# flanglet/kanzi-cpp

Measured on AMD Instinct MI355X. Metric: encode+decode MB/s on the synthetic stand-in for silesia.tar (bit-exact), higher is better.
Workload: dtype u8

## Files before the change

kanzi-cpp_amd/csrc/bwt_fwd.hip:

```cpp
#include "common.hpp"
#include "stages.hpp"
#include "bwt_common.hpp"

#include <cstdlib>
#include <cstring>
#include <algorithm>
#include <cmath>
#include "prims.hpp"
#include <chrono>
#include <vector>

namespace knz {

constexpr u32 SM_TS = 1792;
constexpr u32 SM_WIN = 2048;
constexpr u32 SM_G = 256;
constexpr u32 MED_CAP = 8192;
constexpr u32 MED_LO_CAP = 2048;
constexpr u32 SUPER_CAP = 8192;
constexpr int GATHER_THREADS = 512;
constexpr u32 GATHER_ROWS = 16;
static_assert(MED_CAP <= GATHER_ROWS * GATHER_THREADS, "k_bwt_f_gather_desc judges a medium group from one batch of loads");
constexpr u32 LARGE_OS_MIN = 1000000;
constexpr u32 NO_BIT = 0x7FFFFFFFu;

struct FwdView {
    const u32* base;
    int nBlocks;
    u32 total;
    u32* SA;
    u32* ISA;
    u64* ISA2;
    u32 round;
    u32* K;
    u32* gbits;
    u32* gnew;
    u32* counters;
    const u32* ovr;
    const u32* rtbits;
    uint2* medStage;
    uint2* verdictNow;
    const uint2* verdictWas;
};

constexpr u32 VERDICT_WHOLE = 1, VERDICT_PLAIN = 2;
__host__ __device__ __forceinline__ u32 verdict_word(u32 round, u32 status, u32 members) { return (round << 24) | (status << 16) | members; }
static_assert(MED_CAP < (1u << 16), "verdict_word keeps a medium group's size in 16 bits");

enum FwdCounter : u32 {
    CNT_SMALL_LEFT = 0,
    CNT_MED = 1,
    CNT_LARGE = 2,
    CNT_LARGE_MEMBERS = 3,
    CNT_RUN = 4,
    CNT_RUN_MEMBERS = 5,
    CNT_RUN_LONGEST = 6,
    CNT_SUPER = 7,
    CNT_RUNS = 8,
    CNT_MED_LO = 9,
    CNT_STAT_SMALL = 10,
    CNT_STAT_SMALL_GROUPS = 11,
    CNT_STAT_MED = 12,
    CNT_TIED = 13,
    CNT_PROBE_CAND = 14,
    CNT_LINKED = 14,
    CNT_LINK_TIED = 15,
    CNT_STAT_MED_GROUPS = 16,
    CNT_STAT_UNSPLIT = 17,
    CNT_STAT_UNSPLIT_MEMBERS = 18,
    CNT_STAT_MAJ = 19,
    CNT_STAT_MAJ_MEMBERS = 20,
    CNT_STAT_ASLEEP = 21,
    CNT_STAT_ASLEEP_MEMBERS = 22,
    CNT_ROUND_SLOTS = 24,
    CNT_PROBE_SLOTS = 2,
    CNT_LONGEST_BLOCK = 32,
    CNT_NSYM = 33,
};

constexpr u32 LAB_BITS = 28;
constexpr u64 LAB_MASK = (1ull << LAB_BITS) - 1ull;

__device__ __forceinline__ u32 lab_old(const FwdView& v, u32 q, u32 bb)
{
    if (v.ISA2 == nullptr) return v.ISA[q];
    const u64 e = v.ISA2[q];
    const u32 rel = ((u32)(e >> 56) == v.round && v.round != 0) ? (u32)((e >> LAB_BITS) & LAB_MASK) : (u32)(e & LAB_MASK);
    return bb + rel;
}
__device__ __forceinline__ u32 lab_cur(const FwdView& v, u32 q, u32 bb)
{
    if (v.ISA2 == nullptr) return v.ISA[q];
    return bb + (u32)(v.ISA2[q] & LAB_MASK);
}
__device__ __forceinline__ void lab_set(const FwdView& v, u32 p, u32 bb, u32 lab, u32 was)
{
    if (v.ISA2 == nullptr) { v.ISA[p] = lab; return; }
#ifdef KNZ_EMU
    if (v.round != 0 && lab_old(v, p, bb) != was) {
        fprintf(stderr, "lab_set: round %u position %u: was %u, label %u\n", v.round, p, was, lab_old(v, p, bb));
        abort();
    }
#endif
    const u64 nw = (u64)(lab - bb), ow = (v.round == 0) ? nw : (u64)(was - bb);
    v.ISA2[p] = nw | (ow << LAB_BITS) | ((u64)v.round << 56);
}

__device__ __forceinline__ u32 gather_key(const FwdView& v, u32 gp, u32 h, u32 blkBase, u32 blkEnd)
{
    const u32 q = gp + h;
    return (q < blkEnd) ? lab_old(v, q, blkBase) - blkBase + 1u : 0u;
}

__device__ __forceinline__ void classify_child(const FwdView& v, uint2* __restrict__ medNext, uint2* __restrict__ largeNext, u32 start, u32 size, u32& surv)
{
    if (size > MED_CAP) {
        const u32 at = atomicAdd(&v.counters[CNT_LARGE], 1u);
        largeNext[at] = make_uint2(start, size);
        atomicAdd(&v.counters[CNT_LARGE_MEMBERS], size);
    } else if (size > SM_G) {
        v.medStage[start >> 8] = make_uint2(start, size);
    } else if (size > 1) {
        surv = 1;
    }
}

// ... 1742 lines not shown
}

__global__ __launch_bounds__(256) void k_bwt_f_run_members(const u32* __restrict__ moff, u32 nRuns, u32 M, const u64* __restrict__ sKey, int kbits, int hbits,
                                                           u32 nsym, u64* __restrict__ mkeys)
{
    __shared__ u32 sOff[2048 + 1];
    __shared__ u32 sFirst;
    const u32 j0 = blockIdx.x * 2048u;
    if (j0 >= M) return;
    if (threadIdx.x == 0) {
        u32 lo = 0, hi = nRuns;
        while (hi - lo > 1) { const u32 mid = (lo + hi) >> 1; if (moff[mid] <= j0) lo = mid; else hi = mid; }
        sFirst = lo;
    }
    __syncthreads();
    const u32 k0 = sFirst;
    for (u32 i = threadIdx.x; i <= 2048u; i += 256) sOff[i] = (k0 + i < nRuns) ? moff[k0 + i] : 0xFFFFFFFFu;
    __syncthreads();
#pragma unroll
    for (int q = 0; q < 8; q++) {
        const u32 j = j0 + (u32)q * 256u + threadIdx.x;
        if (j >= M) continue;
        u32 lo = 0, hi = 2048;
        while (hi - lo > 1) { const u32 mid = (lo + hi) >> 1; if (sOff[mid] <= j) lo = mid; else hi = mid; }
        if (sOff[hi] <= j) lo = hi;
        const u32 k = k0 + lo;
        const u64 key = sKey[k];
        const u64 cls = key >> (kbits + 1);
        const bool above = (key >> kbits) & 1ull;
        const u64 Rr = (u64)nsym + (u64)(j - sOff[lo]);
        const u64 hiK = above ? ((1ull << hbits) - 1ull - Rr) : Rr;
        mkeys[j] = (((cls << hbits) | hiK) << 32) | (u64)k;
    }
}

__global__ __launch_bounds__(256) void k_bwt_f_run_expand(const u64* __restrict__ mkeys, u32 M, const u64* __restrict__ sKey, const u32* __restrict__ sE,
                                                          int kbits, int hbits, u64* __restrict__ keys, u32* __restrict__ vals, u32* __restrict__ Rout)
{
    const u32 j = blockIdx.x * 256 + threadIdx.x;
    if (j >= M) return;
    const u64 mk = mkeys[j];
    const u32 k = (u32)mk;
    const u64 ch = mk >> 32;
    const u64 hiK = ch & ((1ull << hbits) - 1ull);
    const u64 rk = sKey[k];
    const bool above = (rk >> kbits) & 1ull;
    const u64 T = rk & ((1ull << kbits) - 1ull);
    const u32 Rr = (u32)(above ? ((1ull << hbits) - 1ull - hiK) : hiK);
    keys[j] = (ch << kbits) | T;
    vals[j] = sE[k] - Rr;
    Rout[j] = Rr;
}

__global__ __launch_bounds__(256) void k_bwt_f_run_flags(const u64* __restrict__ keys, u32 M, unsigned long long* __restrict__ bits64)
{
    const u32 j = blockIdx.x * 256 + threadIdx.x;
    const u64 k = (j < M) ? keys[j] : 0ull;
    u32 klo = (u32)__shfl_up((int)(u32)k, 1u, 64), khi = (u32)__shfl_up((int)(u32)(k >> 32), 1u, 64);
    u64 kp = ((u64)khi << 32) | klo;
    if ((threadIdx.x & 63) == 0 && j > 0 && j < M) kp = keys[j - 1];
    const bool f = (j >= M) || (j == 0) || (k != kp);
    const unsigned long long m = __ballot(f);
    if ((threadIdx.x & 63) == 0) bits64[j >> 6] = m;
}

__global__ __launch_bounds__(256) void k_bwt_f_run_place(FwdView v, const uint2* __restrict__ desc, const u32* __restrict__ loff, u32 M, int kbits, const u64* __restrict__ keys,
                                                         const u32* __restrict__ vals, const u32* __restrict__ bits, const u32* __restrict__ winLastIncl,
                                                         const u32* __restrict__ winFirstInclRev, u32 nWin, uint2* __restrict__ largeNext, const u32* __restrict__ memberR,
                                                         u32* __restrict__ ovr, u32* __restrict__ rtbits, const u32* __restrict__ lbase)
{
    __shared__ SmWindow W;
    __shared__ ClassAgg A;
    const int tid = (int)threadIdx.x;
    const u32 jb = blockIdx.x * 256u;
    const u32 win = jb / SM_WIN, j0 = win * SM_WIN;
    agg_init(A);
    if (tid < 64) {
        const u32 w = bits[(j0 >> 5) + (u32)tid];
        W.bw[tid] = w;
        int pm = w ? (tid * 32 + 31 - __clz((int)w)) : -1;
        u32 sm = w ? (u32)(tid * 32 + __ffs((int)w) - 1) : NO_BIT;
        for (int o = 1; o < 64; o <<= 1) {
            const int t = __shfl_up(pm, (unsigned)o, 64);
            if (tid >= o) pm = t > pm ? t : pm;
            const u32 u = (u32)__shfl_down((int)sm, (unsigned)o, 64);
            if (tid + o < 64) sm = u < sm ? u : sm;
        }
        int pex = __shfl_up(pm, 1u, 64);
        if (tid == 0) pex = -1;
        u32 sex = (u32)__shfl_down((int)sm, 1u, 64);
        if (tid == 63) sex = NO_BIT;
        W.prevSet[tid] = pex;
        W.nextSet[tid] = sex;
    }
    __syncthreads();
    const u32 j = jb + (u32)tid;
    u32 surv = 0, mySlot = 0, hLocal = 0, hSize = 0;
    int hKind = -1;
    bool setBit = false;
    if (j < M) {
        const u32 i = j - j0;
        const u32 w = i >> 5, bit = i & 31;
        const u32 lowmask = (bit == 31) ? 0xFFFFFFFFu : ((2u << bit) - 1u);
        const u32 word = W.bw[w];
        const u32 m = word & lowmask;
        const int si = m ? (int)(w * 32 + 31 - (u32)__clz((int)m)) : W.prevSet[w];
// ... 73 lines not shown
        u32 word = 0, have = 0;
#pragma unroll
        for (u32 k = 0; k < 4; k++) {
            const u32 q = 4 * w + k;
            if (q >= qLo && q < qHi) {
                const u32 rr = q - qLo;
                const u32 r = rr + (rr >= r0 ? 1u : 0u);
                const u32 p = SA[bb + r] - bb;
                word |= (u32)s[p - 1] << (8 * k);
                have |= 1u << k;
            }
        }
        if (have == 0xF && al) reinterpret_cast<u32*>(d)[w] = word;
        else for (u32 k = 0; k < 4; k++) if ((have >> k) & 1) d[4 * w + k] = (u8)(word >> (8 * k));
    }
    if (blockIdx.x == 0 && threadIdx.x == 0) {
        d[hdr] = s[n - 1];
        const u32 st = n / (u32)chunks;
        const u32 step = ((u32)chunks * st == n) ? st : st + 1;
        const u32 logNbChunks = (u32)ilog2_u32((u32)chunks);
        d[0] = (u8)((logNbChunks << 2) | (pIndexSize - 1));
        u32 idx = 1;
        for (int k = 0; k < chunks; k++) {
            const u32 prim = lab_cur(fv, bb + (u32)k * step, bb) - bb;
            for (int sh = (int)(pIndexSize - 1) * 8; sh >= 0; sh -= 8) d[idx++] = (u8)(prim >> sh);
        }
        newLen[b] = hdr + n;
    }
}

__global__ __launch_bounds__(256) void k_bwt_f_med_flags(const uint2* __restrict__ stage, u32 nSlots, u32* __restrict__ flags)
{
    const u32 i = blockIdx.x * 256 + threadIdx.x;
    if (i >= nSlots) return;
    const u32 n = stage[i].y;
    flags[i] = (n != 0 && n <= MED_LO_CAP) ? 1u : 0u;
    flags[nSlots + i] = (n > MED_LO_CAP) ? 1u : 0u;
}

__global__ __launch_bounds__(256) void k_bwt_f_med_compact(uint2* __restrict__ stage, u32 nSlots, const u32* __restrict__ prefix, uint2* __restrict__ medNext,
                                                           u32 at, u32* __restrict__ idxLo, u32 atLo, u32* __restrict__ idxHi, u32 atHi, u32* __restrict__ nLoOut)
{
    const u32 i = blockIdx.x * 256 + threadIdx.x;
    if (i >= nSlots) return;
    const u32 nLo = prefix[nSlots];
    if (i == 0) *nLoOut = nLo;
    const uint2 d = stage[i];
    if (d.y == 0) return;
    const u32 pLo = prefix[i], pHi = prefix[nSlots + i] - nLo, g = at + pLo + pHi;
    medNext[g] = d; stage[i] = make_uint2(0u, 0u);
    if (d.y <= MED_LO_CAP) idxLo[atLo + pLo] = g; else idxHi[atHi + pHi] = g;
}

struct FwdTuning { int nsym; int noRunRound; int runFallback; int stats; int link; int plainLabels; int noPack; int noUnsplitSkip; int noGroupSleep; int noMediumFuse; };
static FwdTuning& fwd_tuning()
{
    static FwdTuning t = [] {
        FwdTuning x; x.nsym = 0; x.noRunRound = 0; x.runFallback = 0; x.stats = 0; x.link = 1; x.plainLabels = 0; x.noPack = 0; x.noUnsplitSkip = 0; x.noGroupSleep = 0; x.noMediumFuse = 0;
        if (getenv("KNZ_BWT_PLAIN_LABELS")) x.plainLabels = 1;
        if (getenv("KNZ_BWT_NO_PACK")) x.noPack = 1;
        if (getenv("KNZ_BWT_NO_UNSPLIT_SKIP")) x.noUnsplitSkip = 1;
        if (getenv("KNZ_BWT_NO_GROUP_SLEEP")) x.noGroupSleep = 1;
        if (getenv("KNZ_BWT_NO_MEDIUM_FUSE")) x.noMediumFuse = 1;
        if (const char* e = getenv("KNZ_BWT_LINK")) x.link = atoi(e);
        if (getenv("KNZ_BWT_STATS")) x.stats = 1;
        if (const char* e = getenv("KNZ_BWT_NSYM")) x.nsym = atoi(e);
        if (getenv("KNZ_BWT_NO_RUN_ROUND")) x.noRunRound = 1;
        if (getenv("KNZ_BWT_RUN_FALLBACK")) x.runFallback = 1;
        return x;
    }();
    return t;
}
int bwt_forward_tune(const char* key, int value)
{
    FwdTuning& t = fwd_tuning();
    if (!strcmp(key, "rs_onesweep")) { prims::rs_onesweep_knob().store(value); return 0; }
    if (!strcmp(key, "bwt_nsym")) t.nsym = value;
    else if (!strcmp(key, "bwt_no_run_round")) t.noRunRound = value;
    else if (!strcmp(key, "bwt_run_fallback")) t.runFallback = value;
    else if (!strcmp(key, "bwt_stats")) t.stats = value;
    else if (!strcmp(key, "bwt_link")) t.link = value;
    else if (!strcmp(key, "bwt_plain_labels")) t.plainLabels = value;
    else if (!strcmp(key, "bwt_no_pack")) t.noPack = value;
    else if (!strcmp(key, "bwt_no_unsplit_skip")) t.noUnsplitSkip = value;
    else if (!strcmp(key, "bwt_no_group_sleep")) t.noGroupSleep = value;
    else if (!strcmp(key, "bwt_no_medium_fuse")) t.noMediumFuse = value;
    else return -1;
    return 0;
}

struct FwdScratch {
    u64* keysA; u64* keysB;
    u32* valsA; u32* valsB;
    u32* SA; u32* ISA; u32* K; u64* ISA2;
    u32* t0; u32* t1; u32* t2; u32* t3;
    u32* gbits; u32* gnew; u32* rtbits; u32* ovr; size_t gbitsWords;
    uint2* med[2]; uint2* medStage; uint2* medVerdict[2]; u32* medFlags; u32* medPrefix; u32* medIdxLo; u32* medIdxHi; size_t medSlots; uint2* descInfo; uint2* large[2]; uint2* runList; uint4* superList; u32* ebits;
    u32* loff; u32* lbase;
    u32* survTile;
    u32* linkedTile;
    u32* base;
    u32* counters;
    u32* seg2;
    void* scanTmp;
    void* rsMem;
    u32* byteHist;
    u32* classTab; u32* rbits; u32* rcount; u32* rprefix;
    u32* runPos; u32* runE; u32* runL; u32* sE; u32* rcnt; u32* moff;
    u64* runKeysA; u64* runKeysB; u64* sKey;
    size_t maxRuns;
};

static size_t fwd_align(size_t x) { return (x + 255) & ~(size_t)255; }

static size_t fwd_carve(u8* p, int nBlocks, size_t total, FwdScratch* w, u32 VS)
{
    u8* q = p;
    auto take = [&](size_t sz) { u8* r = q; q += fwd_align(sz); return r; };
    const size_t maxMed = 2 * (total / (SM_G + 1) + 2), maxLarge = total / (MED_CAP + 1) + 2;
    w->gbitsWords = ((total + 64) / 64 + SM_WIN / 64 + 4) * 2 + 128;
    w->keysA = (u64*)take(8 * total); w->keysB = (u64*)take(8 * total);
    w->valsA = (u32*)take(4 * total); w->valsB = (u32*)take(4 * total);
    w->SA = (u32*)take(4 * total); w->ISA = (u32*)take(4 * total); w->K = (u32*)take(4 * total);
    w->ISA2 = (VS <= (1u << LAB_BITS)) ? (u64*)take(8 * total) : (u64*)nullptr;
    w->t0 = (u32*)take(4 * total); w->t1 = (u32*)take(4 * total); w->t2 = (u32*)take(4 * total); w->t3 = (u32*)take(4 * total);
    w->gbits = (u32*)take(4 * w->gbitsWords);
    w->gnew = (u32*)take(4 * w->gbitsWords);
    w->rtbits = (u32*)take(4 * w->gbitsWords);
    w->ovr = (u32*)take(4 * total);
    w->med[0] = (uint2*)take(8 * maxMed); w->med[1] = (uint2*)take(8 * maxMed);
    w->medSlots = total / 256 + 2;
    w->medStage = (uint2*)take(8 * w->medSlots); w->medFlags = (u32*)take(8 * w->medSlots + 64); w->medPrefix = (u32*)take(8 * w->medSlots + 64);
    w->medIdxLo = (u32*)take(4 * maxMed); w->medIdxHi = (u32*)take(4 * maxMed);
    w->medVerdict[0] = (uint2*)take(16 * w->medSlots); w->medVerdict[1] = w->medVerdict[0] + w->medSlots;
    w->large[0] = (uint2*)take(8 * maxLarge); w->large[1] = (uint2*)take(8 * maxLarge);
    w->runList = (uint2*)take(8 * maxMed);
    w->superList = (uint4*)take(16 * maxMed);
    w->descInfo = (uint2*)take(8 * maxMed);
    w->ebits = (u32*)take(4 * w->gbitsWords);
    w->loff = (u32*)take(4 * (maxMed + 1));
    w->lbase = (u32*)take(4 * (maxMed + 1));
    w->survTile = (u32*)take(4 * (total / SM_TS + 64));
    w->linkedTile = (u32*)take(4 * (total / SM_TS + 64));
    w->base = (u32*)take(4ull * (nBlocks + 2));
    w->counters = (u32*)take(256);
    w->byteHist = (u32*)take(1024ull * (nBlocks + 1));
    w->seg2 = (u32*)take(64);
    w->scanTmp = take(prims::scan_tmp_bytes(total + 16));
    w->rsMem = take(prims::rs_ws_bytes(total, nBlocks + 1));
    w->maxRuns = total / 4 + 64;
    w->classTab = (u32*)take(1024ull * (size_t)nBlocks);
    const size_t rw = total / 32 + SM_WIN / 32 + 136;
    w->rbits = (u32*)take(4 * rw); w->rcount = (u32*)take(4 * rw); w->rprefix = (u32*)take(4 * rw);
    w->runPos = (u32*)take(4 * w->maxRuns); w->runE = (u32*)take(4 * w->maxRuns); w->runL = (u32*)take(4 * w->maxRuns);
    w->sE = (u32*)take(4 * w->maxRuns); w->rcnt = (u32*)take(4 * w->maxRuns); w->moff = (u32*)take(4 * w->maxRuns + 64);
    w->runKeysA = (u64*)take(8 * w->maxRuns); w->runKeysB = (u64*)take(8 * w->maxRuns); w->sKey = (u64*)take(8 * w->maxRuns);
    return (size_t)(q - p);
}

size_t bwt_forward_scratch_bytes(int nBlocks, u32 VS, size_t total)
{
    FwdScratch w;
    return fwd_carve(nullptr, nBlocks, total, &w, VS) + 4096;
}

#define GRID1(n) dim3((unsigned)(((n) + 255) / 256)), dim3(256), 0, s

static int bits_for(u64 n, int lo) { while ((1ull << lo) < n) lo++; return lo; }

struct LinkPlan {
    enum Mode { UNTRIED, TRIAL, ON, APPLIED, OFF } mode = UNTRIED;
    int trials = 0; u32 retryH = 0xFFFFFFFFu;
    bool next(u32 h, u32 survMembers, u32 total, u32 linked, u32 tied, bool stats)
    {
        if (mode == TRIAL || mode == APPLIED) {
            const bool paid = linked >= 4096 && tied < linked / 2;
            mode = paid ? ON : OFF;
            if (!paid) retryH = (trials < 2) ? h * 8 : 0xFFFFFFFFu;
            if (stats) fprintf(stderr, "link step: %u members linked, %u of the windows' members still tied after the round -> %s\n", linked, tied, paid ? "on" : "off");
        }
        if (mode == OFF && h >= retryH) mode = UNTRIED;
        if (mode == UNTRIED && survMembers >= total / 8) { mode = TRIAL; trials++; return true; }
        if (mode == ON && survMembers >= total / 64) { mode = APPLIED; return true; }
        return false;
    }
};

struct FwdSort {
    hipStream_t s; const XfStage& st; u32* hp;
    const FwdTuning tune = fwd_tuning();
    BwtView bv; FwdView v; FwdScratch w; size_t maxTotal;
    prims::RsWs rs1;
    u32 total, medSlots, nTiles; int nsym, pbits, kbits;
    bool groupSleep = false;
    u32 h = 1; int cur = 0;
    u64 *keysFree, *keysFree2;
    bool medFuse = false;
    u32 nMedLo = 0;
    u32 nRun, runElems, surv, nMed, nLarge, largeElems, survMembers;
    LinkPlan link; LinkTrial linkTr; std::chrono::steady_clock::time_point statT;
    int fetch(u32 first, u32 n) { return hipMemcpyAsync(hp + first, w.counters + first, 4 * (size_t)n, hipMemcpyDeviceToHost, s) == hipSuccess && hipStreamSynchronize(s) == hipSuccess ? 0 : -1; }
    void merge_bits() { hipLaunchKernelGGL(k_bwt_f_merge_bits, GRID1(total / 32 + 2), w.gbits, w.gnew, total / 32 + 2); }
    void enable_run_tiebits() { if (!v.rtbits) { hipMemsetAsync(w.rtbits, 0, 4 * w.gbitsWords, s); v.ovr = w.ovr; v.rtbits = w.rtbits; } }
    void compact_medium(uint2* dst, u32 at = 0, u32 atLo = 0)
    {
        KScope ks_("k_bwt_f_med_compact");
        hipLaunchKernelGGL(k_bwt_f_med_flags, GRID1(medSlots), w.medStage, medSlots, w.medFlags);
        prims::launch_scan<prims::SCAN_SUM_EXCL>(s, w.medFlags, w.medPrefix, 2 * (size_t)medSlots, nullptr, w.scanTmp, w.counters + CNT_MED);
        hipLaunchKernelGGL(k_bwt_f_med_compact, GRID1(medSlots), w.medStage, medSlots, w.medPrefix, dst, at, w.medIdxLo, atLo, w.medIdxHi, at - atLo, w.counters + CNT_MED_LO);
    }
    void bounds(u32 n, bool last, const u32* bits = nullptr, u32 len = 0, u32 wordsPerWin = 0)
    {
        if (bits) { KScope ks_("k_bwt_f_r0_winsum"); hipLaunchKernelGGL(k_bwt_f_r0_winsum, GRID1(n), bits, len, n, w.t0, w.t2, wordsPerWin); }
        if (last) { KScope ks_("k_bwt_f_scan_max"); prims::launch_scan<prims::SCAN_MAX_INCL>(s, w.t0, w.t1, n, nullptr, w.scanTmp); }
        KScope ks_("k_bwt_f_scan_min"); prims::launch_scan<prims::SCAN_MIN_INCL>(s, w.t2, w.t3, n, nullptr, w.scanTmp);
    }
    template <class KEY, bool HAS_VAL> int sort_one_segment(u32 n, KEY* ka, KEY* kb, u32* va, u32* vb, int loBit, int hiBit, bool oneRead = true)
    {
        hipLaunchKernelGGL(prims::k_rs_one_segment, dim3(1), dim3(64), 0, s, w.seg2, n);
        prims::rs_launch_layout(s, rs1);
        return prims::rs_sort<KEY, HAS_VAL>(s, rs1, ka, kb, va, vb, (size_t)n, loBit, hiBit, oneRead);
    }
    int setup(void* scratch, size_t scratchBytes, BwtSuffixArrays* sa)
    {
        bv.src = st.src; bv.dst = st.dst; bv.len = st.len; bv.cap = st.cap; bv.VS = st.maxLen; bv.nBlocks = st.nBlocks;
        maxTotal = (size_t)st.nBlocks * bv.VS;
        if (fwd_carve(reinterpret_cast<u8*>(scratch), st.nBlocks, maxTotal, &w, bv.VS) > scratchBytes) return -2;
        { KScope ks_("k_bwt_f_bases"); hipLaunchKernelGGL(k_bwt_bases, dim3(1), dim3(64), 0, s, bv, w.base, st.ok, w.counters + CNT_LONGEST_BLOCK, sa ? 1 : 0); }
        hipMemsetAsync(st.newLen, 0, sizeof(u32) * st.nBlocks, s);
        { KScope ks_("k_bwt_f_r0_hist");
          hipMemsetAsync(w.byteHist, 0, 1024ull * st.nBlocks, s);
          hipLaunchKernelGGL(k_bwt_f_bytehist, dim3(64, (unsigned)st.nBlocks), dim3(256), 0, s, bv, w.base, w.byteHist);
          hipLaunchKernelGGL(k_bwt_f_choose_nsym, dim3(1), dim3(256), 0, s, w.byteHist, st.nBlocks, w.counters + CNT_LONGEST_BLOCK, w.counters + CNT_NSYM); }
        if (hipMemcpyAsync(hp, w.base + st.nBlocks, 4, hipMemcpyDeviceToHost, s) != hipSuccess || fetch(CNT_LONGEST_BLOCK, 2)) return -1;
        total = hp[0];
        if (sa) { sa->SA = w.SA; sa->base = w.base; sa->total = total; }
        if (total == 0) return 0;
        v.base = w.base; v.nBlocks = st.nBlocks; v.total = total; v.SA = w.SA; v.ISA = w.ISA; v.K = w.K; v.ISA2 = (w.ISA2 != nullptr && !tune.plainLabels) ? w.ISA2 : (u64*)nullptr;
        v.round = 0; v.gbits = w.gbits; v.gnew = w.gnew; v.counters = w.counters; v.medStage = w.medStage; v.ovr = nullptr; v.rtbits = nullptr;
        v.verdictNow = nullptr; v.verdictWas = nullptr;
        medSlots = (u32)((size_t)total / 256 + 1); nTiles = (total + SM_TS - 1) / SM_TS;
        survMembers = total;
        hipMemsetAsync(w.medStage, 0, 8ull * w.medSlots, s);
        medFuse = v.ISA2 != nullptr && !tune.noMediumFuse;
        groupSleep = !tune.noUnsplitSkip && !tune.noGroupSleep;
        if (groupSleep) hipMemsetAsync(w.medVerdict[0], 0, 16ull * w.medSlots, s);
        pbits = bits_for(hp[CNT_LONGEST_BLOCK], 1);
        const int fit = (64 - pbits) / 8, want = (hp[CNT_NSYM] == 5u) ? 5 : 4;
        nsym = fit < want ? fit : want;
        if (tune.nsym >= 1) nsym = tune.nsym < fit ? tune.nsym : fit;
// ... 23 lines not shown
            if (pass == 0) { TextSrc src; src.src = bv.src; src.P = nsym; src.pbits = pbits; src.shift = pbits; sortPass(src, pass); }
            else { prims::DigitOfKey<u64> src; src.keys = kin; src.shift = pbits + 8 * pass; src.mask = 255u; sortPass(src, pass); }
            std::swap(kin, kout);
        }
        keysFree = kout; keysFree2 = kin;
    }
    int round0_place()
    {
        hipMemsetAsync(w.gbits, 0xFF, 4 * w.gbitsWords, s); hipMemsetAsync(w.gnew, 0, 4 * w.gbitsWords, s);
        hipMemsetAsync(w.counters, 0, 4 * CNT_ROUND_SLOTS, s);
        { KScope ks_("k_bwt_f_r0_flags"); hipLaunchKernelGGL(k_bwt_f_r0_flags, dim3((total + 256 * R0F_ROWS - 1) / (256 * R0F_ROWS)), dim3(256), 0, s, keysFree2, w.base, st.nBlocks, total, nsym, pbits,
                                                             reinterpret_cast<unsigned long long*>(w.gbits)); }
        bounds(nTiles, true, w.gbits, total, SM_TS / 32);
        kbits = bits_for((u64)bv.VS + 2, 1);
        const bool runRound = (2 * kbits + 1) < 64 && !tune.noRunRound;
        { KScope ks_("k_bwt_f_r0_place");
          hipLaunchKernelGGL(k_bwt_f_r0_place_text, dim3(nTiles), dim3(256), 0, s, bv, v, w.t1, w.t3, nTiles, w.large[cur], keysFree2, nsym, pbits, runRound ? w.runList : (uint2*)nullptr);
          merge_bits(); }
        if (fetch(0, CNT_ROUND_SLOTS)) return -1;
        nRun = hp[CNT_RUN]; runElems = hp[CNT_RUN_MEMBERS];
        return 0;
    }
    int run_fallback()
    {
        { KScope ks_("k_bwt_f_run_fallback"); hipLaunchKernelGGL(k_bwt_f_run_fallback, GRID1(nRun), v, w.runList, nRun, w.med[cur], w.large[cur]); }
        nRun = 0; return fetch(0, CNT_ROUND_SLOTS);
    }
    int run_round()
    {
        if (nRun && ((u64)nRun > (1ull << (64 - (2 * kbits + 1))) || tune.runFallback) && run_fallback()) return -1;
        if (!nRun) return 0;
        const u32 nWin = (total + SM_WIN - 1) / SM_WIN;
        { KScope ks_("k_bwt_f_run_ends"); hipLaunchKernelGGL(k_bwt_f_run_ends, dim3(nWin), dim3(256), 0, s, bv, v, reinterpret_cast<u8*>(w.ebits)); }
        bounds(nWin, false, w.ebits, total, SM_WIN / 32);
        hipMemsetAsync(w.classTab, 0xFF, 1024ull * (size_t)st.nBlocks, s);
        { KScope ks_("k_bwt_f_run_classes"); hipLaunchKernelGGL(k_bwt_f_run_classes, GRID1(nRun), bv, v, w.runList, nRun, w.classTab); }
        { KScope ks_("k_bwt_f_run_len"); hipLaunchKernelGGL(k_bwt_f_run_len, dim3(nWin), dim3(256), 0, s, bv, v, w.ebits, w.t3, nWin, w.K, w.classTab, (u32)nsym,
                                                            reinterpret_cast<unsigned long long*>(w.rbits), w.rcount); }
        const u32 nRW = nWin * (SM_WIN / 32);
        { KScope ks_("k_bwt_f_scan_sum"); prims::launch_scan<prims::SCAN_SUM_EXCL>(s, w.rcount, w.rprefix, nRW, nullptr, w.scanTmp, w.counters + CNT_RUNS); }
        { KScope ks_("k_bwt_f_run_compact"); hipLaunchKernelGGL(k_bwt_f_run_compact, GRID1(nRW), w.rbits, w.rprefix, nRW, w.runPos); }
        if (fetch(CNT_RUN_LONGEST, 3)) return -1;
        const u32 nRuns = hp[CNT_RUNS];
        const int hbits = bits_for((u64)hp[CNT_RUN_LONGEST] + 1, 1) + 1;
        const int rbits = bits_for(nRun, 0), idxBits = bits_for(nRuns, 1);
        if (nRuns == 0 || nRuns > w.maxRuns || rbits + hbits > 32 || idxBits + kbits + 1 + rbits > 64) return run_fallback();
        { KScope ks_("k_bwt_f_large_prefix"); hipLaunchKernelGGL(k_bwt_f_large_prefix, dim3(1), dim3(1024), 0, s, w.runList, nRun, w.loff, w.base, st.nBlocks, w.lbase); }
        { KScope ks_("k_bwt_f_run_table"); hipLaunchKernelGGL(k_bwt_f_run_table, GRID1(nRuns), bv, v, w.runPos, nRuns, w.K, w.classTab, kbits, idxBits, w.runKeysA, w.runE, w.runL); }
        const u64* rkSorted;
        { KScope ks_("k_bwt_f_sort_runs");
          rkSorted = sort_one_segment<u64, false>(nRuns, w.runKeysA, w.runKeysB, nullptr, nullptr, idxBits, idxBits + kbits + 1 + rbits) ? w.runKeysB : w.runKeysA; }
        { KScope ks_("k_bwt_f_run_sorted"); hipLaunchKernelGGL(k_bwt_f_run_sorted, GRID1(nRuns), rkSorted, nRuns, idxBits, w.runE, w.runL, (u32)nsym, w.sE, w.sKey, w.rcnt); }
        { KScope ks_("k_bwt_f_scan_sum"); prims::launch_scan<prims::SCAN_SUM_EXCL>(s, w.rcnt, w.moff, nRuns, nullptr, w.scanTmp); }
        { KScope ks_("k_bwt_f_run_members"); hipLaunchKernelGGL(k_bwt_f_run_members, dim3((runElems + 2047) / 2048), dim3(256), 0, s, w.moff, nRuns, runElems, w.sKey, kbits, hbits,
                                                                (u32)nsym, keysFree); }
        u64* rk; u32* rv = w.valsA;
        { KScope ks_("k_bwt_f_sort_members");
          const int r = sort_one_segment<u64, false>(runElems, keysFree, keysFree2, nullptr, nullptr, 32, 32 + hbits + rbits);
          rk = r ? keysFree : keysFree2;
          hipLaunchKernelGGL(k_bwt_f_run_expand, GRID1(runElems), r ? keysFree2 : keysFree, runElems, w.sKey, w.sE, kbits, hbits, rk, rv, w.valsB); }
        u32* mbits = w.ebits; const u32 nWinM = (runElems + SM_WIN - 1) / SM_WIN;
        { KScope ks_("k_bwt_f_large_flags"); hipLaunchKernelGGL(k_bwt_f_run_flags, dim3(nWinM * (SM_WIN / 256)), dim3(256), 0, s, rk, runElems, reinterpret_cast<unsigned long long*>(mbits)); }
        bounds(nWinM, true, mbits, runElems, SM_WIN / 32);
        { KScope ks_("k_bwt_f_large_place");
          hipMemsetAsync(w.rtbits, 0, 4 * w.gbitsWords, s);
          hipLaunchKernelGGL(k_bwt_f_run_place, dim3((runElems + 255) / 256), dim3(256), 0, s, v, w.runList, w.loff, runElems, hbits + kbits, rk, rv, mbits, w.t1, w.t3, nWinM, w.large[cur],
                             w.valsB, w.ovr, w.rtbits, w.lbase);
          v.ovr = w.ovr; v.rtbits = w.rtbits; }
        { KScope ks_("k_bwt_f_merge_bits"); merge_bits(); }
        return 0;
    }
    int probe()
    {
        u32* probeCand = w.medFlags;
        compact_medium(w.med[cur]);
        { KScope ks_("k_bwt_f_probe"); hipLaunchKernelGGL(k_bwt_f_probe_scan, dim3(256), dim3(256), 0, s, v, w.med[cur], (u32)nsym, v.rtbits, probeCand); }
        if (fetch(0, CNT_ROUND_SLOTS)) return -1;
        surv = hp[CNT_SMALL_LEFT]; nMed = hp[CNT_MED]; nMedLo = hp[CNT_MED_LO]; nLarge = hp[CNT_LARGE]; largeElems = hp[CNT_LARGE_MEMBERS];
        if (const u32 nCand = hp[CNT_PROBE_CAND]) {
            enable_run_tiebits();
            hipMemsetAsync(w.counters, 0, 4 * CNT_PROBE_SLOTS, s);
            { KScope ks_("k_bwt_f_probe");
              hipLaunchKernelGGL(k_bwt_f_probe, dim3(std::min<u32>(nCand, 4096)), dim3(512), 0, s, bv, v, w.med[cur], probeCand, nCand, (u32)nsym, w.med[cur ^ 1], w.large[cur], w.ovr, w.rtbits);
              merge_bits(); }
            compact_medium(w.med[cur], nMed, nMedLo);
            if (fetch(0, CNT_MED_LO + 1)) return -1;
            surv |= hp[CNT_SMALL_LEFT]; nMed += hp[CNT_MED]; nMedLo += hp[CNT_MED_LO];
        }
        if (tune.stats) fprintf(stderr, "after round 0 (nsym %d, total %u): run groups %u (%u members); small left %u, medium %u, large %u (%u members)\n",
                                nsym, total, nRun, runElems, surv, nMed, nLarge, largeElems);
        statT = std::chrono::steady_clock::now();
        return 0;
    }
    void link_step()
    {
        KScope ks_("k_bwt_f_link");
        u32* posflag = w.ebits; u32* linked = w.rbits; u32* rev = w.rcount; u32* sufRev = w.rprefix;
        const bool trial = link.mode == LinkPlan::TRIAL; linkTr.n = 0;
        if (trial) { linkTr.blk[linkTr.n++] = 0; if (st.nBlocks >= 5) linkTr.blk[linkTr.n++] = st.nBlocks / 2; if (st.nBlocks >= 3) linkTr.blk[linkTr.n++] = st.nBlocks - 1; }
        const u32 nW = total / 32 + 1;
        hipMemsetAsync(posflag, 0, 4 * (size_t)nW, s);
        hipMemsetAsync(linked, 0, 4 * ((size_t)nTiles * (SM_TS / 32) + 64), s);
        enable_run_tiebits();
        const u32 nTrial = (u32)std::min<u64>((u64)nTiles, ((u64)bv.VS + SM_TS - 1) / SM_TS + 2);
        const dim3 gridL(trial ? nTrial : nTiles, (unsigned)(linkTr.n ? linkTr.n : 1));
        hipLaunchKernelGGL(k_bwt_f_link_small, gridL, dim3(256), 0, s, v, posflag, linked, tune.stats, 1u, w.linkedTile, linkTr);
        hipLaunchKernelGGL(k_bwt_f_link_zeros, GRID1(nW), posflag, nW, rev);
        prims::launch_scan<prims::SCAN_MIN_INCL>(s, rev, sufRev, nW, nullptr, w.scanTmp);
        hipLaunchKernelGGL(k_bwt_f_link_apply, gridL, dim3(256), 0, s, v, posflag, sufRev, nW, linked, h, w.ovr, w.rtbits, 1u, linkTr);
    }
    void sort_small(bool linked)
    {
        KScope ks_("k_bwt_f_sort_small");
        u32* survTile = tune.link ? w.survTile : nullptr;
        if (v.ISA2 && pbits <= 23 && !tune.noPack) hipLaunchKernelGGL(k_bwt_f_small_fused<true>, dim3(nTiles), dim3(256), 0, s, v, h, survTile, tune.stats);
        else if (v.ISA2) hipLaunchKernelGGL(k_bwt_f_small_fused<false>, dim3(nTiles), dim3(256), 0, s, v, h, survTile, tune.stats);
        else hipLaunchKernelGGL(k_bwt_f_sort_small, dim3(nTiles), dim3(256), 0, s, v, survTile);
        if (linked) hipLaunchKernelGGL(k_bwt_f_link_payoff, dim3(1), dim3(256), 0, s, v, w.linkedTile, w.survTile, nTiles, 1u, w.counters + CNT_LINKED, linkTr);
        if (tune.link) prims::launch_scan<prims::SCAN_SUM_EXCL>(s, w.survTile, w.survTile, nTiles, nullptr, w.scanTmp, w.counters + CNT_TIED);
    }
    void sort_medium()
    {
        const int npass = (kbits + 7) / 8, nxt = cur ^ 1;
        if (medFuse) {
            KScope ks_("k_bwt_f_medium_fused"); const int skip = tune.noUnsplitSkip ? 0 : 1; const u32 nMedHi = nMed - nMedLo;
            const auto fuse256 = tune.stats ? k_bwt_f_medium_fused<256, 8, true> : k_bwt_f_medium_fused<256, 8, false>;
            const auto fuse512 = tune.stats ? k_bwt_f_medium_fused<512, 16, true> : k_bwt_f_medium_fused<512, 16, false>;
            if (nMedLo) hipLaunchKernelGGL(fuse256, dim3(std::min<u32>((nMedLo + 7) / 8 * 8, 2048)), dim3(256), 0, s, v, w.med[cur], w.medIdxLo, nMedLo, h, npass, skip, w.med[nxt], w.large[nxt], w.superList);
            if (nMedHi) hipLaunchKernelGGL(fuse512, dim3(std::min<u32>((nMedHi + 7) / 8 * 8, 1024)), dim3(512), 0, s, v, w.med[cur], w.medIdxHi, nMedHi, h, npass, skip, w.med[nxt], w.large[nxt], w.superList);
        } else { KScope ks_("k_bwt_f_sort_medium"); const dim3 gridM(std::min<u32>(nMed, 8192));
          const auto sort256 = tune.stats ? k_bwt_f_sort_medium<256, 8, true> : k_bwt_f_sort_medium<256, 8, false>;
          const auto sort512 = tune.stats ? k_bwt_f_sort_medium<512, 16, true> : k_bwt_f_sort_medium<512, 16, false>;
          hipLaunchKernelGGL(sort256, gridM, dim3(256), 0, s, v, w.med[cur], nMed, npass, SM_G, w.med[nxt], w.large[nxt], w.descInfo, w.superList);
          hipLaunchKernelGGL(sort512, gridM, dim3(512), 0, s, v, w.med[cur], nMed, npass, MED_LO_CAP, w.med[nxt], w.large[nxt], w.descInfo, w.superList); }
        { KScope ks_("k_bwt_f_super"); hipLaunchKernelGGL(k_bwt_f_super, dim3(std::min<u32>(nMed, 512)), dim3(1024), 0, s, v, w.superList, h, npass, w.med[nxt], w.large[nxt]); }
    }
    template <class KEY> void large_keys()
    {
        { KScope ks_("k_bwt_f_large_prefix"); hipLaunchKernelGGL(k_bwt_f_large_prefix, dim3(1), dim3(1024), 0, s, w.large[cur], nLarge, w.loff, w.base, st.nBlocks, w.lbase); }
        KScope ks_("k_bwt_f_large_keys");
        hipLaunchKernelGGL(k_bwt_f_large_keys<KEY>, GRID1(largeElems), v, w.large[cur], nLarge, w.loff, largeElems, h, kbits, reinterpret_cast<KEY*>(keysFree), w.valsA);
    }
    template <class KEY> void sort_large(int lbits)
// ... 78 lines not shown
```

Baseline: 6659.

## Place BWT run members directly by counting instead of radix sorting them

When the longest run is at most 1023, the expansion of run members no longer generates keys and radix-sorts them. It splits the run list into tiles, histograms run lengths per tile, and scans per-segment column offsets across tiles. Each member's output position is then computed directly and written in sorted order. This removes a full 64-bit segmented sort over all run members, at the cost of several small kernels and scans plus extra scratch for tile column tables. The original sort path is kept as a fallback behind a tuning flag and for longer runs.

```diff
diff --git a/kanzi-cpp_amd/csrc/bwt_fwd.hip b/kanzi-cpp_amd/csrc/bwt_fwd.hip
--- a/kanzi-cpp_amd/csrc/bwt_fwd.hip
+++ b/kanzi-cpp_amd/csrc/bwt_fwd.hip
@@ -72,6 +72,7 @@
     CNT_STAT_MAJ_MEMBERS = 20,
     CNT_STAT_ASLEEP = 21,
     CNT_STAT_ASLEEP_MEMBERS = 22,
+    CNT_RUN_TILES = 23,
     CNT_ROUND_SLOTS = 24,
     CNT_PROBE_SLOTS = 2,
     CNT_LONGEST_BLOCK = 32,
@@ -1920,6 +1921,205 @@
     Rout[j] = Rr;
 }
 
+constexpr u32 RUN_TILE = 1024;
+constexpr u32 RUN_ROWS = RUN_TILE / 64;
+constexpr u32 RUN_DIRECT_LMAX = 1023;
+constexpr u32 RUN_COLS = RUN_DIRECT_LMAX + 1;
+constexpr u32 RUN_CH = 256;
+static_assert(RUN_COLS == 4 * 256 && RUN_CH == 256 && RUN_ROWS % 4 == 0, "the kernels below map columns and rows to 256 threads");
+static inline size_t run_tile_slots(size_t maxRuns) { return 2 * (maxRuns / RUN_TILE + 2); }
+
+struct RunTile { u32 k0, k1, a, slot; bool first, last, multi; };
+__device__ __forceinline__ RunTile run_tile(const u32* __restrict__ tileStart, const u32* __restrict__ segStart, u32 nRuns, u32 t)
+{
+    RunTile r;
+    r.k0 = tileStart[t]; r.k1 = tileStart[t + 1]; r.a = segStart[r.k0];
+    r.first = r.k0 == r.a;
+    r.last = r.k1 >= nRuns || segStart[r.k1] == r.k1;
+    r.multi = !(r.first && r.last);
+    r.slot = (r.k1 - r.k0 == RUN_TILE) ? 2u * ((r.k0 + RUN_TILE - 1) / RUN_TILE) : (r.k0 >= RUN_TILE ? 2u * ((r.k0 - 1) / RUN_TILE) + 1u : 1u);
+    return r;
+}
+
+__global__ __launch_bounds__(256) void k_bwt_f_run_seg_marks(const u64* __restrict__ sKey, u32 nRuns, int kbits, u32* __restrict__ segMark)
+{
+    const u32 k = blockIdx.x * 256 + threadIdx.x;
+    if (k >= nRuns) return;
+    segMark[k] = (k > 0 && (sKey[k] >> kbits) == (sKey[k - 1] >> kbits)) ? 0u : k;
+}
+
+__global__ __launch_bounds__(256) void k_bwt_f_run_tile_marks(const u32* __restrict__ segStart, u32 nRuns, u32* __restrict__ tileMark)
+{
+    const u32 k = blockIdx.x * 256 + threadIdx.x;
+    if (k >= nRuns) return;
+    tileMark[k] = ((k - segStart[k]) % RUN_TILE == 0) ? 1u : 0u;
+}
+
+__global__ __launch_bounds__(256) void k_bwt_f_run_tile_starts(const u32* __restrict__ segStart, const u32* __restrict__ tileIdx, u32 nRuns, u32* __restrict__ tileStart)
+{
+    const u32 k = blockIdx.x * 256 + threadIdx.x;
+    if (k >= nRuns) return;
+    const bool mark = (k - segStart[k]) % RUN_TILE == 0;
+    const u32 t = tileIdx[k];
+    if (mark) tileStart[t] = k;
+    if (k + 1 == nRuns) tileStart[t + (mark ? 1u : 0u)] = nRuns;
+}
+
+__global__ __launch_bounds__(256) void k_bwt_f_run_tile_counts(const u32* __restrict__ tileStart, const u32* __restrict__ segStart, const u32* __restrict__ rcnt, u32 nRuns,
+                                                               const u32* __restrict__ nTilesDev, u32 nsym, u32* __restrict__ colTab)
+{
+    __shared__ u32 hist[RUN_COLS];
+    __shared__ u32 wsum[4];
+    const u32 t = blockIdx.x, tid = threadIdx.x;
+    if (t >= *nTilesDev) return;
+    const RunTile T = run_tile(tileStart, segStart, nRuns, t);
+    if (!T.multi) return;
+    for (u32 i = tid; i < RUN_COLS; i += 256) hist[i] = 0;
+    __syncthreads();
+    for (u32 k = T.k0 + tid; k < T.k1; k += 256) { const u32 L = rcnt[k] + nsym - 1u; atomicAdd(&hist[L < RUN_DIRECT_LMAX ? L : RUN_DIRECT_LMAX], 1u); }
+    __syncthreads();
+    u32 x[4], acc = 0;
+#pragma unroll
+    for (u32 i = 0; i < 4; i++) { x[i] = hist[4 * tid + i]; acc += x[i]; }
+    u32 tot;
+    const u32 incl = prims::sc_block_incl<prims::SCAN_SUM_EXCL>(acc, wsum, &tot);
+    u32 ge = tot - (incl - acc);
+    u32* row = colTab + (size_t)T.slot * RUN_COLS;
+#pragma unroll
+    for (u32 i = 0; i < 4; i++) { row[4 * tid + i] = ge; ge -= x[i]; }
+}
+
+__global__ __launch_bounds__(256) void k_bwt_f_run_tile_scan(const u32* __restrict__ tileStart, const u32* __restrict__ segStart, const u64* __restrict__ sKey, u32 nRuns,
+                                                             const u32* __restrict__ nTilesDev, u32 nsym, int kbits, u32* __restrict__ colTab)
+{
+    __shared__ u32 wsum[4];
+    const u32 t0 = blockIdx.x, tid = threadIdx.x, nT = *nTilesDev;
+    if (t0 >= nT) return;
+    const RunTile T0 = run_tile(tileStart, segStart, nRuns, t0);
+    if (!T0.multi || !T0.first) return;
+    const bool above = ((sKey[T0.a] >> kbits) & 1ull) != 0;
+    u32 A[4] = { 0, 0, 0, 0 };
+    for (u32 t = t0; t < nT; t++) {
+        const RunTile T = run_tile(tileStart, segStart, nRuns, t);
+        const u32* row = colTab + (size_t)T.slot * RUN_COLS;
+#pragma unroll
+        for (u32 c = 0; c < 4; c++) A[c] += row[tid + 256 * c];
+        if (T.last) break;
+    }
+    u32 P[4], carry = 0;
+#pragma unroll
+    for (u32 c = 0; c < 4; c++) {
+        if (tid + 256 * c < nsym) A[c] = 0;
+        u32 tot;
+        P[c] = carry + prims::sc_block_incl<prims::SCAN_SUM_EXCL>(A[c], wsum, &tot);
+        carry += tot;
+    }
+    u32 run[4];
+#pragma unroll
+    for (u32 c = 0; c < 4; c++) run[c] = above ? carry - P[c] : P[c] - A[c];
+    for (u32 t = t0; t < nT; t++) {
+        const RunTile T = run_tile(tileStart, segStart, nRuns, t);
+        u32* row = colTab + (size_t)T.slot * RUN_COLS;
+#pragma unroll
+        for (u32 c = 0; c < 4; c++) { const u32 x = row[tid + 256 * c]; row[tid + 256 * c] = run[c]; run[c] += x; }
+        if (T.last) break;
+    }
+}
+
+__global__ __launch_bounds__(256) void k_bwt_f_run_emit(const u32* __restrict__ tileStart, const u32* __restrict__ segStart, const u32* __restrict__ rcnt,
+                                                        const u32* __restrict__ moff, const u64* __restrict__ sKey, const u32* __restrict__ sE, u32 nRuns, u32 M,
+                                                        const u32* __restrict__ nTilesDev, const u32* __restrict__ colTab, u32 nsym, int kbits, int hbits,
+                                                        u64* __restrict__ keys, u32* __restrict__ vals, u32* __restrict__ Rout)
+{
+    __shared__ u32 cnt[RUN_ROWS][RUN_CH];
+    __shared__ u32 colBase[RUN_CH];
+    __shared__ u32 wsum[4];
+    __shared__ u32 sLmax;
+    const u32 t = blockIdx.x, tid = threadIdx.x;
+    if (t >= *nTilesDev) return;
+    const int lane = lane_id();
+    const u32 wave = tid >> 6;
+    const RunTile T = run_tile(tileStart, segStart, nRuns, t);
+    const u32 nRows = (T.k1 - T.k0 + 63) / 64;
+    const u32 segBase = moff[T.a];
+    const u32 tileMembers = (T.k1 < nRuns ? moff[T.k1] : M) - moff[T.k0];
+    const bool above = ((sKey[T.k0] >> kbits) & 1ull) != 0;
+    const u64 hiAll = (1ull << hbits) - 1ull;
+    u32 Lr[RUN_ROWS / 4], rowMax[RUN_ROWS / 4], e[RUN_ROWS / 4];
+    u64 kb[RUN_ROWS / 4];
+    u32 lmax = 0;
+    if (tid == 0) sLmax = 0;
+#pragma unroll
+    for (u32 q = 0; q < RUN_ROWS / 4; q++) {
+        const u32 k = T.k0 + (wave + 4 * q) * 64 + (u32)lane;
+        Lr[q] = 0; e[q] = 0; kb[q] = 0;
+        if (k < T.k1) {
+            const u64 key = sKey[k];
+            Lr[q] = rcnt[k] + nsym - 1u;
+            if (Lr[q] > RUN_DIRECT_LMAX) Lr[q] = RUN_DIRECT_LMAX;
+            e[q] = sE[k];
+            kb[q] = ((key >> (kbits + 1)) << (hbits + kbits)) | (key & ((1ull << kbits) - 1ull));
+        }
+        rowMax[q] = wave_max(Lr[q]);
+        lmax = rowMax[q] > lmax ? rowMax[q] : lmax;
+    }
+    __syncthreads();
+    if (lane == 0) atomicMax(&sLmax, lmax);
+    __syncthreads();
+    const u32 Lmax = sLmax;
+    u32 carry = 0;
+    for (u32 c0 = nsym; c0 <= Lmax; c0 += RUN_CH) {
+        for (u32 i = tid; i < nRows * RUN_CH; i += 256) (&cnt[0][0])[i] = 0;
+        __syncthreads();
+#pragma unroll
+        for (u32 q = 0; q < RUN_ROWS / 4; q++)
+            if (Lr[q] >= c0) atomicAdd(&cnt[wave + 4 * q][Lr[q] - c0 < RUN_CH ? Lr[q] - c0 : RUN_CH - 1], 1u);
+        __syncthreads();
+#pragma unroll
+        for (u32 q = 0; q < RUN_ROWS / 4; q++) {
+            const u32 row = wave + 4 * q;
+            if (row >= nRows) break;
+            u32 x[4], acc = 0;
+#pragma unroll
+            for (u32 i = 0; i < 4; i++) { x[i] = cnt[row][4 * lane + i]; acc += x[i]; }
+            const u32 incl = wave_incl_scan(acc);
+            const u32 tot = (u32)__shfl((int)incl, 63, 64);
+            u32 ge = tot - (incl - acc);
+#pragma unroll
+            for (u32 i = 0; i < 4; i++) { cnt[row][4 * lane + i] = ge; ge -= x[i]; }
+        }
+        __syncthreads();
+        u32 colRuns = 0;
+        for (u32 row = 0; row < nRows; row++) { const u32 x = cnt[row][tid]; cnt[row][tid] = colRuns; colRuns += x; }
+        if (T.multi) {
+            colBase[tid] = (c0 + tid < RUN_COLS) ? colTab[(size_t)T.slot * RUN_COLS + c0 + tid] : 0u;
+        } else {
+            u32 tot;
+            const u32 P = carry + prims::sc_block_incl<prims::SCAN_SUM_EXCL>(colRuns, wsum, &tot);
+            colBase[tid] = above ? tileMembers - P : P - colRuns;
+            carry += tot;
+        }
+        __syncthreads();
+#pragma unroll
+        for (u32 q = 0; q < RUN_ROWS / 4; q++) {
+            const u32 row = wave + 4 * q;
+            if (row >= nRows) break;
+            const u32 Rend = rowMax[q] < c0 + RUN_CH - 1 ? rowMax[q] : c0 + RUN_CH - 1;
+            for (u32 R = c0; R <= Rend; R++) {
+                const bool alive = Lr[q] >= R;
+                const unsigned long long m = __ballot(alive);
+                const u32 j = segBase + colBase[R - c0] + cnt[row][R - c0] + (u32)__popcll(m & __lanemask_lt());
+                if (alive && j < M) {
+                    keys[j] = kb[q] | ((above ? hiAll - (u64)R : (u64)R) << kbits);
+                    vals[j] = e[q] - R;
+                    Rout[j] = R;
+                }
+            }
+        }
+        __syncthreads();
+    }
+}
+
 __global__ __launch_bounds__(256) void k_bwt_f_run_flags(const u64* __restrict__ keys, u32 M, unsigned long long* __restrict__ bits64)
 {
     const u32 j = blockIdx.x * 256 + threadIdx.x;
@@ -2099,16 +2299,17 @@
     if (d.y <= MED_LO_CAP) idxLo[atLo + pLo] = g; else idxHi[atHi + pHi] = g;
 }
 
-struct FwdTuning { int nsym; int noRunRound; int runFallback; int stats; int link; int plainLabels; int noPack; int noUnsplitSkip; int noGroupSleep; int noMediumFuse; };
+struct FwdTuning { int nsym; int noRunRound; int runFallback; int stats; int link; int plainLabels; int noPack; int noUnsplitSkip; int noGroupSleep; int noMediumFuse; int runSort; };
 static FwdTuning& fwd_tuning()
 {
     static FwdTuning t = [] {
-        FwdTuning x; x.nsym = 0; x.noRunRound = 0; x.runFallback = 0; x.stats = 0; x.link = 1; x.plainLabels = 0; x.noPack = 0; x.noUnsplitSkip = 0; x.noGroupSleep = 0; x.noMediumFuse = 0;
+        FwdTuning x; x.nsym = 0; x.noRunRound = 0; x.runFallback = 0; x.stats = 0; x.link = 1; x.plainLabels = 0; x.noPack = 0; x.noUnsplitSkip = 0; x.noGroupSleep = 0; x.noMediumFuse = 0; x.runSort = 0;
         if (getenv("KNZ_BWT_PLAIN_LABELS")) x.plainLabels = 1;
         if (getenv("KNZ_BWT_NO_PACK")) x.noPack = 1;
         if (getenv("KNZ_BWT_NO_UNSPLIT_SKIP")) x.noUnsplitSkip = 1;
         if (getenv("KNZ_BWT_NO_GROUP_SLEEP")) x.noGroupSleep = 1;
         if (getenv("KNZ_BWT_NO_MEDIUM_FUSE")) x.noMediumFuse = 1;
+        if (const char* e = getenv("KNZ_BWT_RUN_SORT")) x.runSort = atoi(e);
         if (const char* e = getenv("KNZ_BWT_LINK")) x.link = atoi(e);
         if (getenv("KNZ_BWT_STATS")) x.stats = 1;
         if (const char* e = getenv("KNZ_BWT_NSYM")) x.nsym = atoi(e);
@@ -2132,6 +2333,7 @@
     else if (!strcmp(key, "bwt_no_unsplit_skip")) t.noUnsplitSkip = value;
     else if (!strcmp(key, "bwt_no_group_sleep")) t.noGroupSleep = value;
     else if (!strcmp(key, "bwt_no_medium_fuse")) t.noMediumFuse = value;
+    else if (!strcmp(key, "bwt_run_sort")) t.runSort = value;
     else return -1;
     return 0;
 }
@@ -2155,6 +2357,7 @@
     u32* classTab; u32* rbits; u32* rcount; u32* rprefix;
     u32* runPos; u32* runE; u32* runL; u32* sE; u32* rcnt; u32* moff;
     u64* runKeysA; u64* runKeysB; u64* sKey;
+    u32* runTileStart; u32* runColTab;
     size_t maxRuns;
 };
 
@@ -2202,6 +2405,8 @@
     w->runPos = (u32*)take(4 * w->maxRuns); w->runE = (u32*)take(4 * w->maxRuns); w->runL = (u32*)take(4 * w->maxRuns);
     w->sE = (u32*)take(4 * w->maxRuns); w->rcnt = (u32*)take(4 * w->maxRuns); w->moff = (u32*)take(4 * w->maxRuns + 64);
     w->runKeysA = (u64*)take(8 * w->maxRuns); w->runKeysB = (u64*)take(8 * w->maxRuns); w->sKey = (u64*)take(8 * w->maxRuns);
+    w->runTileStart = (u32*)take(4 * w->maxRuns + 64);
+    w->runColTab = (u32*)take(4ull * RUN_COLS * run_tile_slots(w->maxRuns));
     return (size_t)(q - p);
 }
 
@@ -2243,6 +2448,7 @@
     u32 h = 1; int cur = 0;
     u64 *keysFree, *keysFree2;
     bool medFuse = false;
+    bool runDirect = false;
     u32 nMedLo = 0;
     u32 nRun, runElems, surv, nMed, nLarge, largeElems, survMembers;
     LinkPlan link; LinkTrial linkTr; std::chrono::steady_clock::time_point statT;
@@ -2372,13 +2578,32 @@
           rkSorted = sort_one_segment<u64, false>(nRuns, w.runKeysA, w.runKeysB, nullptr, nullptr, idxBits, idxBits + kbits + 1 + rbits) ? w.runKeysB : w.runKeysA; }
         { KScope ks_("k_bwt_f_run_sorted"); hipLaunchKernelGGL(k_bwt_f_run_sorted, GRID1(nRuns), rkSorted, nRuns, idxBits, w.runE, w.runL, (u32)nsym, w.sE, w.sKey, w.rcnt); }
         { KScope ks_("k_bwt_f_scan_sum"); prims::launch_scan<prims::SCAN_SUM_EXCL>(s, w.rcnt, w.moff, nRuns, nullptr, w.scanTmp); }
-        { KScope ks_("k_bwt_f_run_members"); hipLaunchKernelGGL(k_bwt_f_run_members, dim3((runElems + 2047) / 2048), dim3(256), 0, s, w.moff, nRuns, runElems, w.sKey, kbits, hbits,
-                                                                (u32)nsym, keysFree); }
         u64* rk; u32* rv = w.valsA;
-        { KScope ks_("k_bwt_f_sort_members");
-          const int r = sort_one_segment<u64, false>(runElems, keysFree, keysFree2, nullptr, nullptr, 32, 32 + hbits + rbits);
-          rk = r ? keysFree : keysFree2;
-          hipLaunchKernelGGL(k_bwt_f_run_expand, GRID1(runElems), r ? keysFree2 : keysFree, runElems, w.sKey, w.sE, kbits, hbits, rk, rv, w.valsB); }
+        runDirect = !tune.runSort && hp[CNT_RUN_LONGEST] <= RUN_DIRECT_LMAX;
+        if (runDirect) {
+            KScope ks_("k_bwt_f_run_direct");
+            u32* segStart = w.runPos; u32* tileIdx = w.runE;
+            const u32 maxTiles = (u32)std::min<u64>((u64)nRuns, 2ull * nRun + nRuns / RUN_TILE + 1);
+            hipLaunchKernelGGL(k_bwt_f_run_seg_marks, GRID1(nRuns), w.sKey, nRuns, kbits, segStart);
+            prims::launch_scan<prims::SCAN_MAX_INCL>(s, segStart, segStart, nRuns, nullptr, w.scanTmp);
+            hipLaunchKernelGGL(k_bwt_f_run_tile_marks, GRID1(nRuns), segStart, nRuns, tileIdx);
+            prims::launch_scan<prims::SCAN_SUM_EXCL>(s, tileIdx, tileIdx, nRuns, nullptr, w.scanTmp, w.counters + CNT_RUN_TILES);
+            hipLaunchKernelGGL(k_bwt_f_run_tile_starts, GRID1(nRuns), segStart, tileIdx, nRuns, w.runTileStart);
+            if (nRuns > RUN_TILE) {
+                hipLaunchKernelGGL(k_bwt_f_run_tile_counts, dim3(maxTiles), dim3(256), 0, s, w.runTileStart, segStart, w.rcnt, nRuns, w.counters + CNT_RUN_TILES, (u32)nsym, w.runColTab);
+                hipLaunchKernelGGL(k_bwt_f_run_tile_scan, dim3(maxTiles), dim3(256), 0, s, w.runTileStart, segStart, w.sKey, nRuns, w.counters + CNT_RUN_TILES, (u32)nsym, kbits, w.runColTab);
+            }
+            rk = keysFree;
+            hipLaunchKernelGGL(k_bwt_f_run_emit, dim3(maxTiles), dim3(256), 0, s, w.runTileStart, segStart, w.rcnt, w.moff, w.sKey, w.sE, nRuns, runElems, w.counters + CNT_RUN_TILES,
+                               w.runColTab, (u32)nsym, kbits, hbits, rk, rv, w.valsB);
+        } else {
+            { KScope ks_("k_bwt_f_run_members"); hipLaunchKernelGGL(k_bwt_f_run_members, dim3((runElems + 2047) / 2048), dim3(256), 0, s, w.moff, nRuns, runElems, w.sKey, kbits, hbits,
+                                                                    (u32)nsym, keysFree); }
+            KScope ks_("k_bwt_f_sort_members");
+            const int r = sort_one_segment<u64, false>(runElems, keysFree, keysFree2, nullptr, nullptr, 32, 32 + hbits + rbits);
+            rk = r ? keysFree : keysFree2;
+            hipLaunchKernelGGL(k_bwt_f_run_expand, GRID1(runElems), r ? keysFree2 : keysFree, runElems, w.sKey, w.sE, kbits, hbits, rk, rv, w.valsB);
+        }
         u32* mbits = w.ebits; const u32 nWinM = (runElems + SM_WIN - 1) / SM_WIN;
         { KScope ks_("k_bwt_f_large_flags"); hipLaunchKernelGGL(k_bwt_f_run_flags, dim3(nWinM * (SM_WIN / 256)), dim3(256), 0, s, rk, runElems, reinterpret_cast<unsigned long long*>(mbits)); }
         bounds(nWinM, true, mbits, runElems, SM_WIN / 32);
@@ -2407,8 +2632,8 @@
             if (fetch(0, CNT_MED_LO + 1)) return -1;
             surv |= hp[CNT_SMALL_LEFT]; nMed += hp[CNT_MED]; nMedLo += hp[CNT_MED_LO];
         }
-        if (tune.stats) fprintf(stderr, "after round 0 (nsym %d, total %u): run groups %u (%u members); small left %u, medium %u, large %u (%u members)\n",
-                                nsym, total, nRun, runElems, surv, nMed, nLarge, largeElems);
+        if (tune.stats) fprintf(stderr, "after round 0 (nsym %d, total %u): run groups %u (%u members); small left %u, medium %u, large %u (%u members); run members placed directly %u, sorted %u\n",
+                                nsym, total, nRun, runElems, surv, nMed, nLarge, largeElems, (nRun && runDirect) ? runElems : 0u, (nRun && !runDirect) ? runElems : 0u);
         statT = std::chrono::steady_clock::now();
         return 0;
     }
```

Measured after the change: 6941, median of 6. 1.04x the previous value.
